# renegade-fi/renegade

Measured on AMD Instinct MI355X. Metric: VALID MATCH MPC proofs/sec (Intent And Balance Private Settlement), higher is better.
Workload: dtype u256; 1 GPU; intent_and_balance_private_settlement_proof; domain_n=4096, num_public=17, srs_power=13, prover_mode=cohort (lockstep rounds, fused per-round MSMs), total_proofs=4752, parallelism=x1 gpus, cohort=48, 4 in flight

## Files before the change

### renegade_amd/csrc/lagrange_kernels.hip

```cpp
#include <hip/hip_runtime.h>
#include "gpu_curve.hpp"
#include "msm_digits.hpp"

namespace rng {

struct Canon4 {
    uint64_t l[4];
};

__device__ inline G1Jac g1_mul_canon(const G1Jac& p, const uint64_t s[4]) {
    int top = -1;
    for (int i = 3; i >= 0 && top < 0; --i)
        if (s[i]) top = 64 * i + 63 - __clzll((long long)s[i]);
    G1Jac acc = G1Jac::identity();
    for (int bit = top; bit >= 0; --bit) {
        acc = acc.dbl();
        if ((s[bit >> 6] >> (bit & 63)) & 1) acc = acc.add(p);
    }
    return acc;
}

__global__ __launch_bounds__(256) void k_g1_ntt_load(const G1Aff* srs, uint32_t n,
                                                     G1Jac* pts) {
    uint32_t i = blockIdx.x * blockDim.x + threadIdx.x;
    if (i >= n) return;
    pts[i] = G1Jac::from_affine(srs[i]);
}

__global__ __launch_bounds__(64) void k_g1_ntt_pass(G1Jac* pts, uint32_t n, uint32_t h,
                                                    const Fr* tw) {
    uint32_t t = blockIdx.x * blockDim.x + threadIdx.x;
    if (t >= n / 2) return;
    uint32_t blk = t / h, j = t - blk * h;
    uint32_t i0 = blk * 2 * h + j, i1 = i0 + h;
    G1Jac a = pts[i0], b = pts[i1];
    pts[i0] = a.add(b);
    b.Y = b.Y.neg();
    G1Jac d = a.add(b);
    if (j != 0) {
        uint64_t s[4];
        tw[j * (n / (2 * h))].to_canonical(s);
        d = g1_mul_canon(d, s);
    }
    pts[i1] = d;
}

__global__ __launch_bounds__(64) void k_g1_ntt_finish(const G1Jac* in, const G1Aff* srs,
                                                      uint32_t n, uint32_t logn,
                                                      Canon4 ninv, G1Jac* out) {
    uint32_t i = blockIdx.x * blockDim.x + threadIdx.x;
    if (i >= n + 2) return;
    if (i >= n) {
        out[i] = G1Jac::from_affine(srs[i]).madd(srs[i - n], true);
        return;
    }
    uint32_t r = __brev(i) >> (32 - logn);
    out[i] = g1_mul_canon(in[r], ninv.l);
}

constexpr uint32_t LAG_NORM = 8;

__global__ __launch_bounds__(64) void k_g1_normalize(const G1Jac* pts, uint32_t N,
                                                     G1Aff* out, uint32_t* bad) {
    uint32_t t = blockIdx.x * blockDim.x + threadIdx.x;
    uint32_t lo = t * LAG_NORM;
    if (lo >= N) return;
    uint32_t cnt = N - lo < LAG_NORM ? N - lo : LAG_NORM;
    Fq pref[LAG_NORM];
    Fq run = Fq::one();
    for (uint32_t j = 0; j < cnt; ++j) {
        Fq z = pts[lo + j].Z;
        if (z.is_zero()) {
            atomicOr(bad, 1u);
            return;
        }
        run = run.mul(z);
        pref[j] = run;
    }
    Fq inv = run.inverse();
    for (int j = (int)cnt - 1; j >= 0; --j) {
        G1Jac p = pts[lo + j];
        Fq zinv = j ? inv.mul(pref[j - 1]) : inv;
        inv = inv.mul(p.Z);
        Fq zinv2 = zinv.sqr();
        G1Aff a;
        a.x = p.X.mul(zinv2);
        a.y = p.Y.mul(zinv2.mul(zinv));
        out[lo + j] = a;
    }
}


template <typename F>
__device__ inline void msm_signed_digits(const uint64_t s[4], uint32_t c, uint32_t W, F f) {
    uint32_t carry = 0;
    for (uint32_t w = 0; w < W; ++w) {
        MsmDigit d = msm_recode_digit(s, c, w, carry);
        if (d.mag) f(w, d.mag, d.sign);
    }
}

__global__ __launch_bounds__(256) void k_msm_digit_count(const uint64_t* scalars,
                                                         uint32_t total_scalars, uint32_t c,
                                                         uint32_t W, uint32_t* counts) {
    uint32_t idx = blockIdx.x * blockDim.x + threadIdx.x;
    if (idx >= total_scalars) return;
    uint64_t s[4] = {scalars[4 * idx], scalars[4 * idx + 1], scalars[4 * idx + 2],
                     scalars[4 * idx + 3]};
    uint32_t cnt = 0;
    if (s[0] | s[1] | s[2] | s[3])
        msm_signed_digits(s, c, W, [&](uint32_t, uint32_t, uint32_t) { ++cnt; });
    counts[idx] = cnt;
}

__global__ __launch_bounds__(256) void k_msm_digits_compact(
    const uint64_t* scalars, uint32_t n, uint32_t c, uint32_t W, uint32_t B, uint32_t N,
    const uint32_t* offs, uint32_t* keys, uint32_t* vals) {
    uint32_t idx = blockIdx.x * blockDim.x + threadIdx.x;
    if (idx >= n * B) return;
    uint64_t s[4] = {scalars[4 * idx], scalars[4 * idx + 1], scalars[4 * idx + 2],
                     scalars[4 * idx + 3]};
    if (!(s[0] | s[1] | s[2] | s[3])) return;
    uint32_t b = idx / n, i = idx % n;
    uint32_t o = offs[idx];
    msm_signed_digits(s, c, W, [&](uint32_t w, uint32_t mag, uint32_t sign) {
        keys[o] = (b << c) | mag;
        vals[o] = (sign << 31) | (w * N + i);
        ++o;
    });
}

__global__ __launch_bounds__(256) void k_count_nonzero_scalars(const uint64_t* scalars,
                                                               uint32_t total,
                                                               uint32_t* out) {
    uint32_t idx = blockIdx.x * blockDim.x + threadIdx.x;
    bool nz = false;
    if (idx < total)
        nz = (scalars[4 * idx] | scalars[4 * idx + 1] | scalars[4 * idx + 2] |
              scalars[4 * idx + 3]) != 0;
    uint32_t cnt = (uint32_t)__popcll(__ballot(nz));
    if ((threadIdx.x & 63) == 0 && cnt) atomicAdd(out, cnt);
}

__global__ __launch_bounds__(256) void k_lagrange_scalars(const Fr* evals,
                                                          const Fr* blinders, uint32_t n,
                                                          uint64_t total ,
                                                          uint64_t* out) {
    uint64_t i = (uint64_t)blockIdx.x * blockDim.x + threadIdx.x;
    if (i >= total) return;
    uint64_t g = i / (n + 2);
    uint32_t j = (uint32_t)(i - g * (n + 2));
    Fr v = j < n ? evals[g * n + j] : (blinders ? blinders[2 * g + (j - n)] : Fr::zero());
    v.to_canonical(out + 4 * i);
}

}
```

### renegade_amd/csrc/msm_digits.hpp

```cpp
#pragma once
#include <cstdint>

#if defined(__HIPCC__)
#define MSM_DIGIT_HD __host__ __device__
#else
#define MSM_DIGIT_HD
#endif

namespace rng {

struct MsmDigit {
    uint32_t mag;
    uint32_t sign;
};

MSM_DIGIT_HD inline MsmDigit msm_recode_digit(const uint64_t s[4], uint32_t c, uint32_t w,
                                              uint32_t& carry) {
    const uint32_t half = 1u << (c - 1);
    const uint64_t cmask = (1ull << c) - 1;
    const uint32_t bit0 = w * c;
    const uint32_t limb = bit0 >> 6, off = bit0 & 63;
    uint64_t raw = limb < 4 ? s[limb] >> off : 0;
    if (off + c > 64 && limb + 1 < 4) raw |= s[limb + 1] << (64 - off);
    raw = (raw & cmask) + carry;
    MsmDigit d;
    if (raw > half) {
        d.mag = (uint32_t)((1ull << c) - raw);
        d.sign = 1;
        carry = 1;
    } else {
        d.mag = (uint32_t)raw;
        d.sign = 0;
        carry = 0;
    }
    return d;
}

}
```

### renegade_amd/csrc/prover_api.hip

```cpp
#include <array>
#include <atomic>
#include <chrono>
#include <condition_variable>
#include <cstdio>
#include <functional>
#include <cstdlib>
#include <cstring>
#include <map>
#include <memory>
#include <mutex>
#include <stdexcept>
#include <thread>
#include <vector>

#include "../../include/rng_prover.h"
#include "ntt_kernels.hip"
#include "msm_kernels.hip"
#include "lagrange_kernels.hip"
#include "plonk_kernels.hip"
#include "perm_kernels.hip"
#include "open_kernels.hip"
#include "plonk_circuit.hpp"
#include "plonk_host.hpp"
#include "plonk_rounds.hpp"
// ... 39 lines not shown
    struct Job {
        std::function<void(uint32_t)> fn;
        uint32_t count;
        std::atomic<uint32_t> next{0}, done{0};
    };

  public:
    static HostPool& inst() {
        static HostPool* p = new HostPool();
        return *p;
    }

    void parallel_for(uint32_t count, const std::function<void(uint32_t)>& fn) {
        if (count == 0) return;
        if (count == 1 || workers_.empty()) {
            for (uint32_t i = 0; i < count; ++i) fn(i);
            return;
        }
        std::unique_lock<std::mutex> job_lk(job_mu_);
        auto job = std::make_shared<Job>();
        job->fn = fn;
        job->count = count;
        {
            std::lock_guard<std::mutex> lk(mu_);
            job_ = job;
            ++generation_;
        }
        cv_.notify_all();
        run_job(*job);
        {
            std::unique_lock<std::mutex> lk(mu_);
            done_cv_.wait(lk, [&] {
                return job->done.load(std::memory_order_acquire) >= count;
            });
            job_.reset();
        }
    }

  private:
    HostPool() {
        unsigned n = std::thread::hardware_concurrency();
        if (n == 0) n = 4;
        if (n > 32) n = 32;
        for (unsigned t = 0; t + 1 < n; ++t)
            workers_.emplace_back([this] { worker_loop(); });
    }
    void run_job(Job& job) {
        for (;;) {
            uint32_t i = job.next.fetch_add(1, std::memory_order_relaxed);
            if (i >= job.count) break;
            job.fn(i);
            if (job.done.fetch_add(1, std::memory_order_acq_rel) + 1 >= job.count) {
                std::lock_guard<std::mutex> lk(mu_);
                done_cv_.notify_all();
            }
        }
    }
    void worker_loop() {
        uint64_t seen = 0;
        for (;;) {
            std::shared_ptr<Job> job;
            {
                std::unique_lock<std::mutex> lk(mu_);
                cv_.wait(lk, [&] { return generation_ != seen || stopping_; });
                if (stopping_) return;
                seen = generation_;
                job = job_;
            }
            if (job) run_job(*job);
        }
    }
    std::mutex job_mu_;
    std::mutex mu_;
    std::condition_variable cv_, done_cv_;
    std::vector<std::thread> workers_;
    std::shared_ptr<Job> job_;
    uint64_t generation_ = 0;
    bool stopping_ = false;

  public:
    void stop() {
        std::unique_lock<std::mutex> job_lk(job_mu_);
        {
            std::lock_guard<std::mutex> lk(mu_);
            if (stopping_) return;
            stopping_ = true;
        }
        cv_.notify_all();
        for (auto& t : workers_) t.join();
        workers_.clear();
    }
};

struct EvtTimer {
    hipEvent_t ev[8];
    int used = 0;
    EvtTimer() {
        for (auto& e : ev) hipEventCreate(&e);
    }
    ~EvtTimer() {
        for (auto& e : ev) hipEventDestroy(e);
    }
    void mark(hipStream_t s) {
        if (used < 8) hipEventRecord(ev[used++], s);
    }
    void collect(double* out, int n) {
        hipEventSynchronize(ev[used - 1]);
        for (int i = 0; i < n && i + 1 < used; ++i) {
            float ms = 0;
            hipEventElapsedTime(&ms, ev[i], ev[i + 1]);
            out[i] = ms;
        }
    }
};


struct NttPlan {
    uint32_t n, logn, N1, N2, logN1, logN2, split_log;
    Fr *wst1_f = nullptr, *wst2_f = nullptr, *ta_f = nullptr, *tb_f = nullptr;
    Fr *wst1_i = nullptr, *wst2_i = nullptr, *ta_i = nullptr, *tb_i = nullptr;
    Fr ninv;
    Fr* scratch = nullptr;
    uint64_t scratch_elems = 0;
    Fr *gpow = nullptr, *gpow_inv = nullptr, *xpow = nullptr;
};

static Fr h_fr_root_of_unity(uint32_t n) {
    static const u64 root_c[4] = FR_TWO_ADIC_ROOT;
    Fr root = Fr::from_canonical(root_c);
    uint32_t logn = 0;
    while ((1u << logn) < n) logn++;
    for (uint32_t i = logn; i < FR_TWO_ADICITY; ++i) root = root.sqr();
    return root;
}

struct RngCtxImpl {
    std::vector<uint64_t> srs_g1_host;
    uint64_t srs_count = 0;
    void* srs_dev = nullptr;
    struct FixedTable {
        uint32_t c = 0;
        void* dev = nullptr;
    };
    FixedTable fixed_tables[3];
    struct LookupTable {
        void* dev = nullptr;
        bool tried = false;
    };
    LookupTable lookup_tables[3];
    struct LagrangeDomain {
        bool usable = false;
        void* bases = nullptr;
        FixedTable tables[2];
    };
    std::map<uint64_t, LagrangeDomain> lagrange;
    uint64_t h_g2[16];
    uint64_t beta_h_g2[16];
    std::map<uint32_t, std::unique_ptr<NttPlan>> plans;
    std::mutex mu;

    ~RngCtxImpl() {
        for (auto& kv : plans) {
            NttPlan* p = kv.second.get();
            for (Fr* b : {p->wst1_f, p->wst2_f, p->ta_f, p->tb_f, p->wst1_i,
                          p->wst2_i, p->ta_i, p->tb_i, p->scratch, p->gpow,
                          p->gpow_inv, p->xpow})
                hip_free_guarded(b);
        }
        hip_free_guarded(srs_dev);
        for (auto& t : fixed_tables) hip_free_guarded(t.dev);
        for (auto& t : lookup_tables) hip_free_guarded(t.dev);
        for (auto& kv : lagrange) {
            hip_free_guarded(kv.second.bases);
            for (auto& t : kv.second.tables) hip_free_guarded(t.dev);
        }
    }
};

static int build_pow_table(Fr** out, const Fr& base, uint64_t step, uint64_t count) {
    HIP_CHECK(hipMalloc(out, count * sizeof(Fr)));
    uint32_t blocks = (uint32_t)((count + 255) / 256);
    hipLaunchKernelGGL(k_pow_table, dim3(blocks), dim3(256), 0, 0, *out, base, step, count);
    HIP_CHECK(hipGetLastError());
    return RNG_OK;
}

static constexpr uint32_t NTT_SMALL_MAX = 1024;
static constexpr uint64_t NTT_MAX_N = 1ull << 24;
static constexpr bool NTT_FILL_DEFAULT = true;

static bool ntt_args_ok(uint64_t n, uint64_t batch) {
    return n >= 2 && !(n & (n - 1)) && n <= NTT_MAX_N && batch >= 1;
}

static NttPlan* get_plan(RngCtxImpl* ctx, uint32_t n, uint64_t batch) {
    std::lock_guard<std::mutex> lk(ctx->mu);
    auto it = ctx->plans.find(n);
    NttPlan* p;
    if (it != ctx->plans.end()) {
        p = it->second.get();
    } else {
        auto np = std::make_unique<NttPlan>();
        p = np.get();
        p->n = n;
        p->logn = 0;
        while ((1u << p->logn) < n) p->logn++;
        p->logN2 = p->logn / 2;
        p->logN1 = p->logn - p->logN2;
        p->N1 = 1u << p->logN1;
        p->N2 = 1u << p->logN2;
        p->split_log = p->logN2 < 6 ? p->logN2 : 6;
        Fr w = h_fr_root_of_unity(n);
        Fr wi = w.inverse();
        Fr wN1_f = w.pow_u64(p->N2), wN2_f = w.pow_u64(p->N1);
        Fr wN1_i = wi.pow_u64(p->N2), wN2_i = wi.pow_u64(p->N1);
        uint64_t split = 1ull << p->split_log;
        if (n <= NTT_SMALL_MAX) {
            if (build_pow_table(&p->wst1_f, w, 1, n / 2) != RNG_OK) return nullptr;
            if (build_pow_table(&p->wst1_i, wi, 1, n / 2) != RNG_OK) return nullptr;
        } else {
            if (build_pow_table(&p->wst1_f, wN1_f, 1, p->N1 / 2) != RNG_OK) return nullptr;
            if (build_pow_table(&p->wst2_f, wN2_f, 1, p->N2 / 2) != RNG_OK) return nullptr;
            if (build_pow_table(&p->ta_f, w, split, (uint64_t)p->N1 * (p->N2 >> p->split_log)) != RNG_OK) return nullptr;
            if (build_pow_table(&p->tb_f, w, 1, (uint64_t)p->N1 * split) != RNG_OK) return nullptr;
            if (build_pow_table(&p->wst1_i, wN1_i, 1, p->N1 / 2) != RNG_OK) return nullptr;
            if (build_pow_table(&p->wst2_i, wN2_i, 1, p->N2 / 2) != RNG_OK) return nullptr;
            if (build_pow_table(&p->ta_i, wi, split, (uint64_t)p->N1 * (p->N2 >> p->split_log)) != RNG_OK) return nullptr;
            if (build_pow_table(&p->tb_i, wi, 1, (uint64_t)p->N1 * split) != RNG_OK) return nullptr;
        }
        u64 nc[4] = {n, 0, 0, 0};
        p->ninv = Fr::from_canonical(nc).inverse();
        if (hipDeviceSynchronize() != hipSuccess) return nullptr;
        ctx->plans.emplace(n, std::move(np));
    }
    if (n > NTT_SMALL_MAX && p->scratch_elems < (uint64_t)n * batch) {
        if (p->scratch) hipFree(p->scratch);
        if (hipMalloc(&p->scratch, (uint64_t)n * batch * sizeof(Fr)) != hipSuccess) {
            p->scratch = nullptr;
            p->scratch_elems = 0;
            return nullptr;
        }
        p->scratch_elems = (uint64_t)n * batch;
    }
    return p;
}

static int ntt_dev_run(RngCtxImpl* ctx, Fr* data, Fr* out, uint32_t n, uint64_t batch,
                       bool inverse, hipStream_t stream = 0) {
    NttPlan* p = get_plan(ctx, n, 0);
    if (!p) return RNG_ERR_HIP;
    if (n <= NTT_SMALL_MAX) {
        Fr* wst = inverse ? p->wst1_i : p->wst1_f;
        hipLaunchKernelGGL(k_ntt_small, dim3((uint32_t)batch), dim3(512), n * sizeof(Fr),
                           stream, data, wst, n, p->logn, p->ninv, inverse ? 1 : 0);
        HIP_CHECK(hipGetLastError());
        if (out != data)
            HIP_CHECK(hipMemcpyAsync(out, data, (uint64_t)n * batch * sizeof(Fr),
                                     hipMemcpyDeviceToDevice, stream));
        return RNG_OK;
    }
    Fr* wst1 = inverse ? p->wst1_i : p->wst1_f;
    Fr* wst2 = inverse ? p->wst2_i : p->wst2_f;
    Fr* ta = inverse ? p->ta_i : p->ta_f;
    Fr* tb = inverse ? p->tb_i : p->tb_f;
    static uint32_t pw_lds_cap = [] {
        const char* e = getenv("RNG_NTT_PAIR_LDS");
        return e ? (uint32_t)atoi(e) : 65536u;
    }();
    static const bool fill = [] {
        const char* e = getenv("RNG_NTT_FILL");
        return e ? atoi(e) != 0 : NTT_FILL_DEFAULT;
    }();
    const uint32_t fpw1 = NTT_FILL_ELEMS / p->N2, fpw2 = NTT_FILL_ELEMS / p->N1;
    const bool fill1 = fill && fpw1 >= 2 && fpw1 <= p->N1;
    const bool fill2 = fill && fpw2 >= 2 && fpw2 <= p->N2;
    const uint32_t pw1 = (2u * p->N2 * sizeof(Fr) <= pw_lds_cap) ? 2 : 1;
    const uint32_t pw2 = (2u * p->N1 * sizeof(Fr) <= pw_lds_cap) ? 2 : 1;
    uint32_t lds1 = pw1 * p->N2 * sizeof(Fr);
    uint32_t lds2 = pw2 * p->N1 * sizeof(Fr);
    EvtTimer et;
    et.mark(stream);
    if (fill1)
        hipLaunchKernelGGL(k_ntt_col_fill, dim3((uint32_t)(p->N1 / fpw1 * batch)),
                           dim3(NTT_FILL_THREADS), NTT_FILL_ELEMS * sizeof(Fr), stream, data,
                           wst2, ta, tb, p->N1, p->N2, p->logN2, p->split_log,
                           (uint32_t)__builtin_ctz(fpw1));
    else if (pw1 == 2)
        hipLaunchKernelGGL(k_ntt_col<2>, dim3((uint32_t)(p->N1 / 2 * batch)), dim3(512),
                           lds1, stream, data, wst2, ta, tb, p->N1, p->N2, p->logN2,
                           p->split_log);
    else
        hipLaunchKernelGGL(k_ntt_col<1>, dim3((uint32_t)(p->N1 * batch)), dim3(512),
                           lds1, stream, data, wst2, ta, tb, p->N1, p->N2, p->logN2,
                           p->split_log);
    HIP_CHECK(hipGetLastError());
    et.mark(stream);
    if (fill2)
        hipLaunchKernelGGL(k_ntt_row_fill, dim3((uint32_t)(p->N2 / fpw2 * batch)),
                           dim3(NTT_FILL_THREADS), NTT_FILL_ELEMS * sizeof(Fr), stream, data,
                           out, wst1, p->N1, p->N2, p->logN1, (uint32_t)__builtin_ctz(fpw2),
                           p->ninv, inverse ? 1 : 0);
    else if (pw2 == 2)
        hipLaunchKernelGGL(k_ntt_row<2>, dim3((uint32_t)(p->N2 / 2 * batch)), dim3(512),
                           lds2, stream, data, out, wst1, p->N1, p->N2, p->logN1,
                           p->ninv, inverse ? 1 : 0);
    else
        hipLaunchKernelGGL(k_ntt_row<1>, dim3((uint32_t)(p->N2 * batch)), dim3(512),
                           lds2, stream, data, out, wst1, p->N1, p->N2, p->logN1,
                           p->ninv, inverse ? 1 : 0);
    HIP_CHECK(hipGetLastError());
    et.mark(stream);
    et.collect(tls_ntt_times, 2);
    return RNG_OK;
}


struct MsmEnv {
    int fixed;
    int c;
    int chunk;
    int subb;
    int seg_cap;
    int debug;
    int lookup;
    int lookup_max_mb;
    int lookup_c;
    int lookup_l;
};

static const MsmEnv& msm_env() {
    static const MsmEnv env = [] {
        auto get = [](const char* name, int unset) {
            const char* e = getenv(name);
            return e ? atoi(e) : unset;
        };
        return MsmEnv{get("RNG_MSM_FIXED", 1),  get("RNG_MSM_C", 0),
                      get("RNG_MSM_CHUNK", 0),  get("RNG_MSM_SUBB", 0),
                      get("RNG_MSM_SEGCAP", 0), get("RNG_MSM_DEBUG", 0),
                      get("RNG_MSM_LOOKUP", -1), get("RNG_MSM_LOOKUP_MAX_MB", 10240),
                      get("RNG_MSM_LOOKUP_C", 0), get("RNG_MSM_LOOKUP_L", 0)};
    }();
    return env;
}

struct ProverEnv {
    int z_device;
    int r1_lagrange;
    int open_device;
    int cohort_trace;
    static bool on(int v, bool path_default) { return v < 0 ? path_default : v == 1; }
};

static const ProverEnv& prover_env() {
    static const ProverEnv env = [] {
        auto tri = [](const char* name) {
            const char* e = getenv(name);
            return e ? (atoi(e) != 0 ? 1 : 0) : -1;
        };
        const char* t = getenv("RNG_COHORT_TRACE");
        return ProverEnv{tri("RNG_Z_DEVICE"), tri("RNG_R1_LAGRANGE"), tri("RNG_OPEN_DEVICE"),
                         t ? atoi(t) : 0};
    }();
    return env;
}

struct MsmBases {
    const G1Aff* points;
    uint64_t table_stride;
    static MsmBases plain(const G1Aff* bases) { return {bases, 0}; }
    static MsmBases table(const G1Aff* t, uint64_t stride) { return {t, stride}; }
    bool fixed() const { return table_stride != 0; }
};

struct MsmShape {
    uint64_t n;
    uint32_t B, c;
    bool fixed;
    bool compact;
    uint32_t Wd;
    uint32_t W;
    uint32_t G;
    uint32_t key_shift;
    uint64_t total;
    uint64_t nb;
    uint32_t chunk_sz;
    uint64_t nchunks;
    uint32_t cw;
    uint32_t subb;
    uint32_t seg_cap;
    uint32_t sentinel;
    uint32_t sort_bits;
};

static MsmShape msm_shape(uint64_t n, uint32_t B, uint32_t c, bool fixed,
                          bool compact = false) {
    const MsmEnv& env = msm_env();
    MsmShape sh;
    sh.n = n;
    sh.B = B;
    sh.c = c;
    sh.fixed = fixed;
    sh.compact = compact;
    sh.Wd = (256 + c - 1) / c;
    sh.W = fixed ? 1 : sh.Wd;
    sh.G = B * sh.W;
    sh.key_shift = fixed ? c : 16;
    sh.total = n * B * sh.Wd;
    sh.nb = (1ull << (c - 1)) * sh.G;
    sh.chunk_sz = MSM_CHUNK;
    while (sh.chunk_sz > 2 && sh.nb / sh.chunk_sz < 131072) sh.chunk_sz >>= 1;
    if (env.chunk >= 2 && env.chunk <= 16) sh.chunk_sz = (uint32_t)env.chunk;
    if ((1u << (c - 1)) < sh.chunk_sz) sh.chunk_sz = 1u << (c - 1);
    sh.nchunks = ((1ull << (c - 1)) / sh.chunk_sz) * sh.G;
    sh.cw = (1u << (c - 1)) / sh.chunk_sz;
    sh.subb = MSM_SUBB;
    while (sh.subb > 1 && sh.cw / sh.subb < 64) sh.subb >>= 1;
    while (sh.subb < 256 && sh.G * sh.subb < 4096 && sh.cw / (2 * sh.subb) >= 64 &&
           (uint64_t)sh.G * sh.subb * 2 <= 8192)
        sh.subb <<= 1;
    if (env.subb >= 1 && env.subb <= 256) sh.subb = (uint32_t)env.subb;
    sh.seg_cap = msm_seg_cap(sh.total);
    if (fixed && env.seg_cap >= 8 && env.seg_cap <= (int)MSM_MAX_SEG)
        sh.seg_cap = (uint32_t)env.seg_cap;
    uint32_t gb = 1;
    while ((1u << gb) <= sh.G) ++gb;
    sh.sentinel = sh.G << sh.key_shift;
    sh.sort_bits = sh.key_shift + gb;
    return sh;
}

struct MsmScratch {
    uint32_t *keys_in = nullptr, *keys_out = nullptr, *vals_in = nullptr, *vals_out = nullptr;
    void* sort_temp = nullptr;
    size_t sort_temp_bytes = 0;
    uint8_t* head_flags = nullptr;
    uint32_t* heads = nullptr;
    uint32_t* lens = nullptr;
    uint32_t* nsub = nullptr;
    uint32_t* sub_off = nullptr;
    uint32_t* sub_start = nullptr;
    uint32_t* sub_len = nullptr;
    uint32_t* sub_len_sorted = nullptr;
    uint32_t* sub_order = nullptr;
    uint32_t* nsub_sorted = nullptr;
    uint32_t* head_order = nullptr;
    G1Jac* partials2 = nullptr;
    uint32_t* head_count = nullptr;
    void* select_temp = nullptr;
    size_t select_temp_bytes = 0;
    void* scan_temp = nullptr;
    size_t scan_temp_bytes = 0;
    G1Jac* buckets = nullptr;
    G1Jac* partials = nullptr;
    G1Jac* window_sums = nullptr;
    uint64_t window_sums_cap = 0;
    G1Jac* result = nullptr;
    uint64_t cap_entries = 0;
    uint64_t cap_nb = 0;
    uint64_t cap_nchunks = 0;
    uint64_t last_entries = 0;

    ~MsmScratch() {
        for (void* b : {(void*)keys_in, (void*)keys_out, (void*)vals_in, (void*)vals_out,
                        sort_temp, (void*)head_flags, (void*)heads, (void*)lens,
                        (void*)nsub, (void*)sub_off, (void*)sub_start, (void*)sub_len,
                        (void*)sub_len_sorted, (void*)sub_order,
                        (void*)nsub_sorted, (void*)head_order,
                        (void*)partials2, (void*)head_count, select_temp, scan_temp,
                        (void*)buckets, (void*)partials, (void*)window_sums,
                        (void*)result})
            hip_free_guarded(b);
    }
};

static thread_local std::unique_ptr<MsmScratch> tls_msm_scratch;

static int msm_scratch_ensure(const MsmShape& sh, hipStream_t stream, MsmScratch** out) {
    if (!tls_msm_scratch) tls_msm_scratch = std::make_unique<MsmScratch>();
    MsmScratch* s = tls_msm_scratch.get();
    if (s->cap_entries < sh.total || s->cap_nb < sh.nb || s->cap_nchunks < sh.nchunks) {
        uint64_t cap_total = sh.total + sh.total / 2 + 64;
        uint64_t cap_nb2 = sh.nb + sh.nb / 2 + 64;
        uint64_t cap_nch = sh.nchunks + sh.nchunks / 2 + 64;
        if (cap_total < s->cap_entries) cap_total = s->cap_entries;
        if (cap_nb2 < s->cap_nb) cap_nb2 = s->cap_nb;
        if (cap_nch < s->cap_nchunks) cap_nch = s->cap_nchunks;
        tls_msm_scratch = std::make_unique<MsmScratch>();
        s = tls_msm_scratch.get();
        HIP_CHECK(hipMalloc(&s->keys_in, cap_total * 4));
        HIP_CHECK(hipMalloc(&s->keys_out, cap_total * 4));
        HIP_CHECK(hipMalloc(&s->vals_in, cap_total * 4));
        HIP_CHECK(hipMalloc(&s->vals_out, cap_total * 4));
        rocprim::radix_sort_pairs(nullptr, s->sort_temp_bytes, s->keys_in, s->keys_out,
// ... 376 lines not shown
    tls_msm_times[2] = ms;
    MsmShape sh{};
    sh.B = sh.G = B;
    sh.W = 1;
    sh.subb = bpp;
    sh.c = c;
    msm_host_fold(sh, wsums, h_result);
    return RNG_OK;
}

static int msm_srs_run(RngCtxImpl* ctx, const uint64_t* d_canon, uint64_t m, uint32_t B,
                       G1Jac* res, int window_c = 0, int mode = 0) {
    if (m == 0 || m > ctx->srs_count || B == 0) return RNG_ERR_BAD_ARG;
    const int c_env = msm_env().c;
    if (window_c == 0 && c_env >= 8 && c_env <= 16) window_c = c_env;
    if (window_c != 0 && (window_c < 8 || window_c > 16)) return RNG_ERR_BAD_ARG;
    if (mode == 3 || (mode == 0 && msm_fixed_enabled() && msm_lookup_wanted(B))) {
        uint32_t c = (uint32_t)window_c;
        const G1Aff* table = nullptr;
        if (B <= 65535)
            table = window_c ? msm_lookup_table(ctx, c) : msm_lookup_select(ctx, &c);
        if (table) return msm_lookup_run(table, ctx->srs_count, d_canon, m, c, res, B);
        if (mode == 3) return RNG_ERR_BAD_ARG;
    }
    if (mode == 1 || (mode == 0 && msm_fixed_enabled())) {
        uint32_t c = window_c ? (uint32_t)window_c : msm_fixed_c(m, B);
        uint32_t gb = 1;
        while ((1u << gb) <= B) ++gb;
        const G1Aff* table = (c + gb <= 32) ? msm_fixed_table(ctx, c) : nullptr;
        if (table)
            return msm_dev_run(MsmBases::table(table, ctx->srs_count), d_canon, m, c, res,
                               B);
        if (mode == 1) return RNG_ERR_BAD_ARG;
    }
    uint32_t c = window_c ? (uint32_t)window_c : msm_auto_c(m);
    if ((uint64_t)B * ((256 + c - 1) / c) > 60000) return RNG_ERR_BAD_ARG;
    return msm_dev_run(MsmBases::plain((const G1Aff*)ctx->srs_dev), d_canon, m, c, res, B);
}


constexpr int MSM_LAGRANGE_UNUSABLE = -100;

static int lagrange_build_bases(RngCtxImpl* ctx, uint64_t n, void** out_bases) {
    const uint32_t N = (uint32_t)n + 2;
    uint32_t logn = 0;
    while ((1ull << logn) < n) ++logn;
    const hipStream_t st = RNG_STREAM;
    G1Jac *pts = nullptr, *fin = nullptr;
    Fr* tw = nullptr;
    uint32_t* bad = nullptr;
    void* bases = nullptr;
    auto cleanup = [&] {
        hipFree(pts);
        hipFree(fin);
        hipFree(tw);
        hipFree(bad);
    };
    if (hipMalloc(&pts, n * sizeof(G1Jac)) != hipSuccess ||
        hipMalloc(&fin, (uint64_t)N * sizeof(G1Jac)) != hipSuccess ||
        hipMalloc(&tw, (n / 2) * sizeof(Fr)) != hipSuccess ||
        hipMalloc(&bad, 4) != hipSuccess ||
        hipMalloc(&bases, (uint64_t)N * sizeof(G1Aff)) != hipSuccess) {
        cleanup();
        hipFree(bases);
        return RNG_ERR_HIP;
    }
    const Fr winv = h_fr_root_of_unity((uint32_t)n).inverse();
    Fr nfr = Fr::one();
    for (uint32_t i = 0; i < logn; ++i) nfr = nfr.add(nfr);
    Canon4 ninv;
    nfr.inverse().to_canonical(ninv.l);
    const G1Aff* srs = (const G1Aff*)ctx->srs_dev;
    hipMemsetAsync(bad, 0, 4, st);
    hipLaunchKernelGGL(k_pow_table, dim3((uint32_t)((n / 2 + 255) / 256)), dim3(256), 0, st,
                       tw, winv, (uint64_t)1, n / 2);
    hipLaunchKernelGGL(k_g1_ntt_load, dim3((uint32_t)((n + 255) / 256)), dim3(256), 0, st,
                       srs, (uint32_t)n, pts);
    for (uint32_t h = (uint32_t)n / 2; h >= 1; h >>= 1)
        hipLaunchKernelGGL(k_g1_ntt_pass, dim3((uint32_t)((n / 2 + 63) / 64)), dim3(64), 0,
                           st, pts, (uint32_t)n, h, (const Fr*)tw);
    hipLaunchKernelGGL(k_g1_ntt_finish, dim3((N + 63) / 64), dim3(64), 0, st,
                       (const G1Jac*)pts, srs, (uint32_t)n, logn, ninv, fin);
    const uint32_t norm_threads = (N + LAG_NORM - 1) / LAG_NORM;
    hipLaunchKernelGGL(k_g1_normalize, dim3((norm_threads + 63) / 64), dim3(64), 0, st,
                       (const G1Jac*)fin, N, (G1Aff*)bases, bad);
    uint32_t h_bad = 1;
    bool ok = hipGetLastError() == hipSuccess &&
              hipMemcpyAsync(&h_bad, bad, 4, hipMemcpyDeviceToHost, st) == hipSuccess &&
              hipStreamSynchronize(st) == hipSuccess;
    cleanup();
    if (!ok || h_bad) {
        hipFree(bases);
        return ok ? MSM_LAGRANGE_UNUSABLE : RNG_ERR_HIP;
    }
    *out_bases = bases;
    return RNG_OK;
}

static const G1Aff* msm_lagrange_table(RngCtxImpl* ctx, uint64_t n, uint32_t c) {
    if (!ctx->srs_dev || n < 2 || (n & (n - 1)) || n > (1ull << 28) ||
        n + 2 > ctx->srs_count || c < 8 || c > 16)
        return nullptr;
    const uint64_t N = n + 2;
    const uint32_t W = (256 + c - 1) / c;
    if ((uint64_t)W * N * sizeof(G1Aff) > (1ull << 30)) return nullptr;
    static const int trace = msm_env().debug;
    std::lock_guard<std::mutex> lk(ctx->mu);
    auto it = ctx->lagrange.find(n);
    if (it == ctx->lagrange.end()) {
        auto t0 = std::chrono::steady_clock::now();
        RngCtxImpl::LagrangeDomain dom;
        dom.usable = lagrange_build_bases(ctx, n, &dom.bases) == RNG_OK;
        it = ctx->lagrange.emplace(n, dom).first;
        if (trace)
            fprintf(stderr, "[lagrange] n=%lu bases %s in %.2f ms\n", (unsigned long)n,
                    dom.usable ? "built" : "UNUSABLE",
                    std::chrono::duration<double, std::milli>(
                        std::chrono::steady_clock::now() - t0).count());
    }
    RngCtxImpl::LagrangeDomain& dom = it->second;
    if (!dom.usable) return nullptr;
    for (auto& t : dom.tables)
        if (t.dev && t.c == c) return (const G1Aff*)t.dev;
    for (auto& t : dom.tables) {
        if (t.dev) continue;
        auto t0 = std::chrono::steady_clock::now();
        void* dev = nullptr;
        if (hipMalloc(&dev, (uint64_t)W * N * sizeof(G1Aff)) != hipSuccess) return nullptr;
        hipLaunchKernelGGL(k_msm_fixed_table, dim3((uint32_t)((N + 255) / 256)), dim3(256),
                           0, RNG_STREAM, (const G1Aff*)dom.bases, (uint32_t)N, c, W,
                           (G1Aff*)dev);
        if (hipGetLastError() != hipSuccess ||
            hipStreamSynchronize(RNG_STREAM) != hipSuccess) {
            hipFree(dev);
            return nullptr;
        }
        t.c = c;
        t.dev = dev;
        if (trace)
            fprintf(stderr, "[lagrange] n=%lu c=%u table (%.1f MB) in %.2f ms\n",
                    (unsigned long)n, c, (double)W * N * sizeof(G1Aff) / 1e6,
                    std::chrono::duration<double, std::milli>(
                        std::chrono::steady_clock::now() - t0).count());
        return (const G1Aff*)dev;
    }
    return nullptr;
}

constexpr uint32_t MSM_LAGRANGE_SPARSE_C = 8, MSM_LAGRANGE_DENSE_C = 13;
static uint32_t msm_lagrange_c(uint64_t n, uint32_t B, uint64_t nonzero) {
    return nonzero * 2 <= (uint64_t)B * n ? MSM_LAGRANGE_SPARSE_C : 0;
}

static int msm_lagrange_run(RngCtxImpl* ctx, uint64_t n, const uint64_t* d_canon, uint32_t B,
                            G1Jac* res, int window_c = 0, bool dense_too = false) {
    if (n < 2 || (n & (n - 1)) || B == 0 || !d_canon) return RNG_ERR_BAD_ARG;
    if (n + 2 > ctx->srs_count) return MSM_LAGRANGE_UNUSABLE;
    const int c_env = msm_env().c;
    if (window_c == 0 && c_env >= 8 && c_env <= 16) window_c = c_env;
    if (window_c != 0 && (window_c < 8 || window_c > 16)) return RNG_ERR_BAD_ARG;
    uint32_t c = (uint32_t)window_c;
    if (c == 0) {
        MsmScratch* s = nullptr;
        int rc = msm_scratch_ensure(msm_shape(n + 2, B, 8, true, true), RNG_STREAM, &s);
        if (rc != RNG_OK) return rc;
        const uint32_t ns = (uint32_t)(B * (n + 2));
        uint32_t nz = 0;
        HIP_CHECK(hipMemsetAsync(s->head_count, 0, 4, RNG_STREAM));
        hipLaunchKernelGGL(k_count_nonzero_scalars, dim3((ns + 255) / 256), dim3(256), 0,
                           RNG_STREAM, d_canon, ns, s->head_count);
        HIP_CHECK(hipGetLastError());
        HIP_CHECK(hipMemcpyAsync(&nz, s->head_count, 4, hipMemcpyDeviceToHost, RNG_STREAM));
        HIP_CHECK(hipStreamSynchronize(RNG_STREAM));
        c = msm_lagrange_c(n, B, nz);
        if (c == 0) {
            if (!dense_too) return MSM_LAGRANGE_UNUSABLE;
            c = MSM_LAGRANGE_DENSE_C;
        }
    }
    uint32_t gb = 1;
    while ((1u << gb) <= B) ++gb;
    if (c + gb > 32) return MSM_LAGRANGE_UNUSABLE;
    const G1Aff* table = msm_lagrange_table(ctx, n, c);
    if (!table) return MSM_LAGRANGE_UNUSABLE;
    return msm_dev_run(MsmBases::table(table, n + 2), d_canon, n + 2, c, res, B, RNG_STREAM,
                       true);
}

constexpr uint32_t R1_LAGRANGE_MIN_K = 2;


static int ensure_coset_tables(RngCtxImpl* ctx, NttPlan* p) {
    std::lock_guard<std::mutex> lk(ctx->mu);
    if (p->gpow) return RNG_OK;
    uint32_t m = p->n;
    Fr g = Fr::from_u64(FR_GENERATOR);
    Fr gi = g.inverse();
    if (build_pow_table(&p->gpow, g, 1, m) != RNG_OK) return RNG_ERR_HIP;
    if (build_pow_table(&p->gpow_inv, gi, 1, m) != RNG_OK) return RNG_ERR_HIP;
    Fr wm = h_fr_root_of_unity(m);
    if (build_pow_table(&p->xpow, wm, 1, m) != RNG_OK) return RNG_ERR_HIP;
    uint32_t blocks = (m + 255) / 256;
    hipLaunchKernelGGL(k_scale_const, dim3(blocks), dim3(256), 0, 0, p->xpow, g, m);
    HIP_CHECK(hipGetLastError());
    HIP_CHECK(hipDeviceSynchronize());
    return RNG_OK;
}

static int coset_fwd_dev(RngCtxImpl* ctx, Fr* in, Fr* out, uint32_t m) {
    NttPlan* p = get_plan(ctx, m, 1);
    if (!p) return RNG_ERR_HIP;
    if (ensure_coset_tables(ctx, p) != RNG_OK) return RNG_ERR_HIP;
    uint32_t blocks = (m + 255) / 256;
    hipLaunchKernelGGL(k_mul_pointwise, dim3(blocks), dim3(256), 0, RNG_STREAM, in,
                       p->gpow, m);
    HIP_CHECK(hipGetLastError());
    return ntt_dev_run(ctx, in, out, m, 1, false, RNG_STREAM);
}

struct ProveScratch {
    static constexpr uint32_t SLOTS = 13;
    uint64_t n = 0;
    Fr* tmp = nullptr;
    Fr* stage = nullptr;
    uint64_t* canon = nullptr;
    ~ProveScratch() {
        for (void* b : {(void*)tmp, (void*)stage, (void*)canon}) hip_free_guarded(b);
    }
};

struct PlonkPkImpl : PlonkPkHost {
    Fr* sel_coset = nullptr;
    Fr* sig_coset = nullptr;
    Fr* l1_coset = nullptr;
    Fr* sig_evals_dev = nullptr;
    Fr* wpow_dev = nullptr;
    Fr* coef_dev = nullptr;
    RngCtxImpl* ctx = nullptr;
    ~PlonkPkImpl() {
        for (void* b : {(void*)sel_coset, (void*)sig_coset, (void*)l1_coset,
                        (void*)sig_evals_dev, (void*)wpow_dev, (void*)coef_dev})
            hip_free_guarded(b);
    }
};

static thread_local std::unique_ptr<ProveScratch> tls_prove_scratch;

static int prove_scratch_ensure(uint64_t n) {
    if (tls_prove_scratch && tls_prove_scratch->n >= n) return RNG_OK;
    tls_prove_scratch = std::make_unique<ProveScratch>();
    ProveScratch* s = tls_prove_scratch.get();
    HIP_CHECK(hipMalloc(&s->tmp, 8 * n * sizeof(Fr)));
    HIP_CHECK(hipMalloc(&s->stage, ProveScratch::SLOTS * (n + 3) * sizeof(Fr)));
    HIP_CHECK(hipMalloc(&s->canon, ProveScratch::SLOTS * 4 * (n + 3) * 8));
    s->n = n;
    return RNG_OK;
}


constexpr bool Z_DEVICE_DEFAULT = true;

static void perm_product_host(const PlonkPkImpl& pk, const Fr& w, const Fr* wires,
                              const Fr& beta, const Fr& gamma, Fr* ze) {
    const uint64_t n = pk.n;
    std::vector<Fr> znum(n), zden(n);
    Fr wi = Fr::one();
    for (uint64_t i = 0; i < n; ++i) {
        Fr num = Fr::one(), den = Fr::one();
        for (int j = 0; j < 5; ++j) {
            Fr wv = wires[(size_t)j * n + i];
            num = num.mul(wv.add(beta.mul(pk.k[j]).mul(wi)).add(gamma));
            den = den.mul(wv.add(beta.mul(pk.sig_evals[j][i])).add(gamma));
        }
        znum[i] = num;
        zden[i] = den;
        wi = wi.mul(w);
    }
    std::vector<Fr> zden_inv = hbatch_inverse(zden);
    ze[0] = Fr::one();
    for (uint64_t i = 1; i < n; ++i) ze[i] = ze[i - 1].mul(znum[i - 1]).mul(zden_inv[i - 1]);
}

struct PermScratch {
    Fr* dev = nullptr;
    Fr* tile_tot = nullptr;
    Fr* tile_pre = nullptr;
    Fr* totals = nullptr;
    Fr* qinv = nullptr;
    Fr* bg = nullptr;
    std::vector<Fr> h_bg, h_q;
    ~PermScratch() { hip_free_guarded(dev); }
};

static thread_local std::unique_ptr<PermScratch> tls_perm_scratch;

static PermScratch* perm_scratch_get() {
    if (tls_perm_scratch) return tls_perm_scratch.get();
    auto s = std::make_unique<PermScratch>();
    const size_t tiles = (size_t)2 * PERM_MAX_BATCH * PERM_MAX_TILES;
    const size_t elems = 2 * tiles + 5 * (size_t)PERM_MAX_BATCH;
    if (hipMalloc(&s->dev, elems * sizeof(Fr)) != hipSuccess) return nullptr;
    s->tile_tot = s->dev;
    s->tile_pre = s->tile_tot + tiles;
    s->totals = s->tile_pre + tiles;
    s->qinv = s->totals + 2 * PERM_MAX_BATCH;
    s->bg = s->qinv + PERM_MAX_BATCH;
    s->h_bg.resize(2 * PERM_MAX_BATCH);
    s->h_q.resize(PERM_MAX_BATCH);
    tls_perm_scratch = std::move(s);
    return tls_perm_scratch.get();
}

static int perm_product_dev(const Fr* wires, const Fr* sigma, const Fr* wpow,
                            const Fr k5[5], const Fr* bg, uint64_t n64, uint64_t batch64,
// ... 1669 lines not shown
```

Before: 3507 proofs/s.

## Add entry-lookup MSM path for sparse round-one Lagrange commitments

Adds a new MSM path for sparse Lagrange-basis commitments. Each nonzero signed digit is looked up in a precomputed multiples table indexed by (window row, magnitude) and mixed-added directly, which removes bucket sorting and bucket reduction. The digit count and the nonzero-density check are fused into one kernel with block-level atomics, so a separate count pass is no longer needed. The cost is a large cached lookup table in device memory, an extra host sync, and a host-side fold of per-block partial sums.

New measurement: 3800 proofs/s (median of 6 runs). 1.08x the previous value.

```diff
diff --git a/renegade_amd/csrc/lagrange_kernels.hip b/renegade_amd/csrc/lagrange_kernels.hip
--- a/renegade_amd/csrc/lagrange_kernels.hip
+++ b/renegade_amd/csrc/lagrange_kernels.hip
@@ -100,6 +100,17 @@
     }
 }
 
+__device__ inline void block_count_add(bool flag, uint32_t* out) {
+    __shared__ uint32_t wave_cnt[4];
+    const uint32_t cnt = (uint32_t)__popcll(__ballot(flag));
+    if ((threadIdx.x & 63) == 0) wave_cnt[threadIdx.x >> 6] = cnt;
+    __syncthreads();
+    if (threadIdx.x == 0) {
+        const uint32_t sum = wave_cnt[0] + wave_cnt[1] + wave_cnt[2] + wave_cnt[3];
+        if (sum) atomicAdd(out, sum);
+    }
+}
+
 __global__ __launch_bounds__(256) void k_msm_digit_count(const uint64_t* scalars,
                                                          uint32_t total_scalars, uint32_t c,
                                                          uint32_t W, uint32_t* counts) {
@@ -113,6 +124,21 @@
     counts[idx] = cnt;
 }
 
+__global__ __launch_bounds__(256) void k_msm_digit_count_density(
+    const uint64_t* scalars, uint32_t total_scalars, uint32_t c, uint32_t W, uint32_t* counts,
+    uint32_t* nonzero) {
+    uint32_t idx = blockIdx.x * blockDim.x + threadIdx.x;
+    uint32_t cnt = 0;
+    if (idx < total_scalars) {
+        uint64_t s[4] = {scalars[4 * idx], scalars[4 * idx + 1], scalars[4 * idx + 2],
+                         scalars[4 * idx + 3]};
+        if (s[0] | s[1] | s[2] | s[3])
+            msm_signed_digits(s, c, W, [&](uint32_t, uint32_t, uint32_t) { ++cnt; });
+    }
+    if (idx <= total_scalars) counts[idx] = cnt;
+    block_count_add(cnt != 0, nonzero);
+}
+
 __global__ __launch_bounds__(256) void k_msm_digits_compact(
     const uint64_t* scalars, uint32_t n, uint32_t c, uint32_t W, uint32_t B, uint32_t N,
     const uint32_t* offs, uint32_t* keys, uint32_t* vals) {
@@ -124,8 +150,8 @@
     uint32_t b = idx / n, i = idx % n;
     uint32_t o = offs[idx];
     msm_signed_digits(s, c, W, [&](uint32_t w, uint32_t mag, uint32_t sign) {
-        keys[o] = (b << c) | mag;
-        vals[o] = (sign << 31) | (w * N + i);
+        keys[o] = msm_entry_key(b, mag, c);
+        vals[o] = msm_entry_val(w, N, i, sign);
         ++o;
     });
 }
@@ -138,8 +164,37 @@
     if (idx < total)
         nz = (scalars[4 * idx] | scalars[4 * idx + 1] | scalars[4 * idx + 2] |
               scalars[4 * idx + 3]) != 0;
-    uint32_t cnt = (uint32_t)__popcll(__ballot(nz));
-    if ((threadIdx.x & 63) == 0 && cnt) atomicAdd(out, cnt);
+    block_count_add(nz, out);
+}
+
+__global__ __launch_bounds__(256) void k_msm_entry_lookup_sum(
+    const uint32_t* keys, const uint32_t* vals, const uint32_t* offs, uint32_t N, uint32_t c,
+    const G1Aff* table, G1Jac* partials) {
+    __shared__ G1Jac red[256];
+    const uint32_t b = blockIdx.y;
+    const uint32_t lo = offs[(uint64_t)b * N], hi = offs[(uint64_t)(b + 1) * N];
+    const uint32_t first = blockIdx.x * 256;
+    G1Jac* out = partials + (uint64_t)b * gridDim.x + blockIdx.x;
+    if (first >= hi - lo) {
+        if (threadIdx.x == 0) *out = G1Jac::identity();
+        return;
+    }
+    const uint32_t active = hi - lo - first < 256 ? hi - lo - first : 256;
+    const uint64_t step = (uint64_t)gridDim.x * 256;
+    G1Jac acc = G1Jac::identity();
+    for (uint64_t e = (uint64_t)lo + first + threadIdx.x; e < hi; e += step) {
+        const uint32_t key = keys[e], val = vals[e];
+        const G1Aff p = table[msm_lookup_index(key, val, c)];
+        acc = acc.madd(p, msm_entry_sign(val) != 0);
+    }
+    red[threadIdx.x] = acc;
+    __syncthreads();
+    for (uint32_t stride = 128; stride > 0; stride >>= 1) {
+        if (threadIdx.x < stride && threadIdx.x + stride < active)
+            red[threadIdx.x] = red[threadIdx.x].add(red[threadIdx.x + stride]);
+        __syncthreads();
+    }
+    if (threadIdx.x == 0) *out = red[0];
 }
 
 __global__ __launch_bounds__(256) void k_lagrange_scalars(const Fr* evals,
diff --git a/renegade_amd/csrc/msm_digits.hpp b/renegade_amd/csrc/msm_digits.hpp
--- a/renegade_amd/csrc/msm_digits.hpp
+++ b/renegade_amd/csrc/msm_digits.hpp
@@ -36,4 +36,28 @@
     return d;
 }
 
+
+MSM_DIGIT_HD inline uint32_t msm_entry_key(uint32_t poly, uint32_t mag, uint32_t c) {
+    return (poly << c) | mag;
 }
+MSM_DIGIT_HD inline uint32_t msm_entry_val(uint32_t w, uint32_t N, uint32_t i, uint32_t sign) {
+    return (sign << 31) | (w * N + i);
+}
+MSM_DIGIT_HD inline uint32_t msm_entry_mag(uint32_t key, uint32_t c) {
+    return key & ((1u << c) - 1);
+}
+MSM_DIGIT_HD inline uint32_t msm_entry_row(uint32_t val) { return val & 0x7fffffffu; }
+MSM_DIGIT_HD inline uint32_t msm_entry_sign(uint32_t val) { return val >> 31; }
+
+MSM_DIGIT_HD inline uint64_t msm_table_rows(uint64_t N, uint32_t c) {
+    return (uint64_t)((256 + c - 1) / c) * N;
+}
+MSM_DIGIT_HD inline bool msm_entry_rows_fit(uint64_t N, uint32_t c) {
+    return msm_table_rows(N, c) < (1ull << 31);
+}
+
+MSM_DIGIT_HD inline uint64_t msm_lookup_index(uint32_t key, uint32_t val, uint32_t c) {
+    return ((uint64_t)msm_entry_row(val) << (c - 1)) + (msm_entry_mag(key, c) - 1);
+}
+
+}
diff --git a/renegade_amd/csrc/prover_api.hip b/renegade_amd/csrc/prover_api.hip
--- a/renegade_amd/csrc/prover_api.hip
+++ b/renegade_amd/csrc/prover_api.hip
@@ -215,6 +215,7 @@
         bool usable = false;
         void* bases = nullptr;
         FixedTable tables[2];
+        LookupTable lookup[3];
     };
     std::map<uint64_t, LagrangeDomain> lagrange;
     uint64_t h_g2[16];
@@ -236,6 +237,7 @@
         for (auto& kv : lagrange) {
             hip_free_guarded(kv.second.bases);
             for (auto& t : kv.second.tables) hip_free_guarded(t.dev);
+            for (auto& t : kv.second.lookup) hip_free_guarded(t.dev);
         }
     }
 };
@@ -389,6 +391,8 @@
     int lookup_max_mb;
     int lookup_c;
     int lookup_l;
+    int r1_lookup;
+    int r1_lookup_s;
 };
 
 static const MsmEnv& msm_env() {
@@ -401,7 +405,8 @@
                       get("RNG_MSM_CHUNK", 0),  get("RNG_MSM_SUBB", 0),
                       get("RNG_MSM_SEGCAP", 0), get("RNG_MSM_DEBUG", 0),
                       get("RNG_MSM_LOOKUP", -1), get("RNG_MSM_LOOKUP_MAX_MB", 10240),
-                      get("RNG_MSM_LOOKUP_C", 0), get("RNG_MSM_LOOKUP_L", 0)};
+                      get("RNG_MSM_LOOKUP_C", 0), get("RNG_MSM_LOOKUP_L", 0),
+                      get("RNG_R1_LOOKUP", -1), get("RNG_R1_LOOKUP_S", 0)};
     }();
     return env;
 }
@@ -1084,6 +1089,188 @@
     return nonzero * 2 <= (uint64_t)B * n ? MSM_LAGRANGE_SPARSE_C : 0;
 }
 
+
+constexpr bool R1_LOOKUP_DEFAULT = true;
+
+static bool r1_lookup_wanted(uint32_t B) {
+    const int sw = msm_env().r1_lookup;
+    return msm_lookup_wanted(B) && (sw < 0 ? R1_LOOKUP_DEFAULT : sw == 1);
+}
+
+static const G1Aff* msm_lagrange_lookup_table(RngCtxImpl* ctx, uint64_t n, uint32_t c) {
+    if (c < MSM_LOOKUP_MIN_C || c > MSM_LOOKUP_MAX_C) return nullptr;
+    const uint64_t N = n + 2;
+    const uint64_t bytes = msm_lookup_bytes(N, c);
+    const int max_mb = msm_env().lookup_max_mb;
+    if (max_mb <= 0 || bytes > ((uint64_t)max_mb << 20) || !msm_entry_rows_fit(N, c))
+        return nullptr;
+    {
+        std::lock_guard<std::mutex> lk(ctx->mu);
+        auto it = ctx->lagrange.find(n);
+        if (it != ctx->lagrange.end()) {
+            RngCtxImpl::LookupTable& t = it->second.lookup[c - MSM_LOOKUP_MIN_C];
+            if (t.dev || t.tried || !it->second.usable) return (const G1Aff*)t.dev;
+        }
+    }
+    const G1Aff* fixed = msm_lagrange_table(ctx, n, c);
+    if (!fixed) return nullptr;
+    std::lock_guard<std::mutex> lk(ctx->mu);
+    RngCtxImpl::LookupTable& t = ctx->lagrange.find(n)->second.lookup[c - MSM_LOOKUP_MIN_C];
+    if (t.dev || t.tried) return (const G1Aff*)t.dev;
+    t.tried = true;
+    size_t free_b = 0, total_b = 0;
+    if (hipMemGetInfo(&free_b, &total_b) != hipSuccess || bytes > free_b / 2) return nullptr;
+    const auto t0 = std::chrono::steady_clock::now();
+    void* dev = nullptr;
+    if (hipMalloc(&dev, bytes) != hipSuccess) {
+        (void)hipGetLastError();
+        return nullptr;
+    }
+    const uint64_t rows = msm_table_rows(N, c);
+    hipLaunchKernelGGL(k_msm_lookup_table, dim3((uint32_t)((rows + 255) / 256)), dim3(256), 0,
+                       RNG_STREAM, fixed, rows, c, (G1Aff*)dev);
+    if (hipGetLastError() != hipSuccess || hipStreamSynchronize(RNG_STREAM) != hipSuccess) {
+        hipFree(dev);
+        return nullptr;
+    }
+    if (msm_env().debug)
+        fprintf(stderr,
+                "[msm] lagrange lookup table n=%lu c=%u rows=%lu bytes=%lu build_ms=%.1f\n",
+                (unsigned long)n, c, (unsigned long)rows, (unsigned long)bytes,
+                std::chrono::duration<double, std::milli>(std::chrono::steady_clock::now() - t0)
+                    .count());
+    t.dev = dev;
+    return (const G1Aff*)dev;
+}
+
+struct R1LookupScratch {
+    uint32_t *counts = nullptr, *offs = nullptr;
+    uint64_t cap_scalars = 0;
+    void* scan_temp = nullptr;
+    size_t scan_temp_bytes = 0;
+    uint32_t *keys = nullptr, *vals = nullptr;
+    uint64_t cap_entries = 0;
+    G1Jac* partials = nullptr;
+    uint64_t cap_partials = 0;
+    ~R1LookupScratch() {
+        for (void* b : {(void*)counts, (void*)offs, scan_temp, (void*)keys, (void*)vals,
+                        (void*)partials})
+            hip_free_guarded(b);
+    }
+};
+static thread_local R1LookupScratch tls_r1_lookup;
+
+static int r1_scratch_grow(void** buf, uint64_t* cap, uint64_t want, size_t elem) {
+    if (*cap >= want) return RNG_OK;
+    hipFree(*buf);
+    *buf = nullptr;
+    *cap = 0;
+    const uint64_t ncap = want + want / 2 + 64;
+    HIP_CHECK(hipMalloc(buf, ncap * elem));
+    *cap = ncap;
+    return RNG_OK;
+}
+
+constexpr uint32_t R1_LOOKUP_PER_LANE = 4, R1_LOOKUP_MAX_S = 64;
+static uint32_t r1_lookup_blocks(uint64_t entries, uint32_t B) {
+    const int s_env = msm_env().r1_lookup_s;
+    if (s_env >= 1 && s_env <= (int)R1_LOOKUP_MAX_S) return (uint32_t)s_env;
+    const uint64_t per_block = 256ull * R1_LOOKUP_PER_LANE;
+    uint64_t S = (entries / B + per_block - 1) / per_block;
+    return (uint32_t)(S < 1 ? 1 : S > R1_LOOKUP_MAX_S ? R1_LOOKUP_MAX_S : S);
+}
+
+constexpr int R1_LOOKUP_DENSE = -101, R1_LOOKUP_NO_TABLE = -102;
+
+static int r1_lookup_run(RngCtxImpl* ctx, uint64_t n, const uint64_t* d_canon, uint32_t B,
+                         uint32_t c, bool gate, G1Jac* h_result) {
+    const hipStream_t stream = RNG_STREAM;
+    const uint32_t N = (uint32_t)n + 2, W = (256 + c - 1) / c;
+    const uint32_t ns = B * N;
+    {
+        std::lock_guard<std::mutex> lk(ctx->mu);
+        auto it = ctx->lagrange.find(n);
+        if (it != ctx->lagrange.end()) {
+            const RngCtxImpl::LookupTable& t = it->second.lookup[c - MSM_LOOKUP_MIN_C];
+            if (!it->second.usable || (t.tried && !t.dev)) return R1_LOOKUP_NO_TABLE;
+        }
+    }
+    R1LookupScratch& s = tls_r1_lookup;
+    if (s.cap_scalars < ns) {
+        uint64_t cap_c = s.cap_scalars, cap_o = s.cap_scalars;
+        int rc = r1_scratch_grow((void**)&s.counts, &cap_c, (uint64_t)ns + 2, 4);
+        if (rc == RNG_OK) rc = r1_scratch_grow((void**)&s.offs, &cap_o, (uint64_t)ns + 2, 4);
+        s.cap_scalars = 0;
+        if (rc != RNG_OK) return rc;
+        hipFree(s.scan_temp);
+        s.scan_temp = nullptr;
+        (void)rocprim::exclusive_scan(nullptr, s.scan_temp_bytes, s.counts, s.offs, 0u, cap_c,
+                                      rocprim::plus<uint32_t>(), stream);
+        HIP_CHECK(hipMalloc(&s.scan_temp, s.scan_temp_bytes));
+        s.cap_scalars = cap_c - 2;
+    }
+    EvtTimer et;
+    et.mark(stream);
+    HIP_CHECK(hipMemsetAsync(s.offs + ns + 1, 0, 4, stream));
+    hipLaunchKernelGGL(k_msm_digit_count_density, dim3(ns / 256 + 1), dim3(256), 0, stream,
+                       d_canon, ns, c, W, s.counts, s.offs + ns + 1);
+    HIP_CHECK(hipGetLastError());
+    (void)rocprim::exclusive_scan(s.scan_temp, s.scan_temp_bytes, s.counts, s.offs, 0u,
+                                  (size_t)ns + 1, rocprim::plus<uint32_t>(), stream);
+    et.mark(stream);
+    uint32_t back[2] = {0, 0};
+    HIP_CHECK(hipMemcpyAsync(back, s.offs + ns, 8, hipMemcpyDeviceToHost, stream));
+    HIP_CHECK(hipStreamSynchronize(stream));
+    const uint64_t entries = back[0];
+    if (gate && msm_lagrange_c(n, B, back[1]) == 0) return R1_LOOKUP_DENSE;
+    const G1Aff* table = msm_lagrange_lookup_table(ctx, n, c);
+    if (!table) return R1_LOOKUP_NO_TABLE;
+    const uint32_t S = r1_lookup_blocks(entries, B);
+    if (msm_env().debug)
+        fprintf(stderr, "[msm] n=%lu B=%u entry-lookup c=%u S=%u entries=%lu (compacted)\n",
+                (unsigned long)N, B, c, S, (unsigned long)entries);
+    for (double& t : tls_msm_times) t = 0;
+    if (entries == 0) {
+        for (uint32_t b = 0; b < B; ++b) h_result[b] = G1Jac::identity();
+        et.collect(tls_msm_times, 1);
+        return RNG_OK;
+    }
+    const uint64_t np = (uint64_t)B * S;
+    int rc = r1_scratch_grow((void**)&s.partials, &s.cap_partials, np, sizeof(G1Jac));
+    if (rc != RNG_OK) return rc;
+    if (s.cap_entries < entries) {
+        uint64_t cap_k = s.cap_entries, cap_v = s.cap_entries;
+        rc = r1_scratch_grow((void**)&s.keys, &cap_k, entries, 4);
+        if (rc == RNG_OK) rc = r1_scratch_grow((void**)&s.vals, &cap_v, entries, 4);
+        s.cap_entries = rc == RNG_OK ? cap_k : 0;
+        if (rc != RNG_OK) return rc;
+    }
+    et.mark(stream);
+    hipLaunchKernelGGL(k_msm_digits_compact, dim3((ns + 255) / 256), dim3(256), 0, stream,
+                       d_canon, N, c, W, B, N, s.offs, s.keys, s.vals);
+    HIP_CHECK(hipGetLastError());
+    et.mark(stream);
+    hipLaunchKernelGGL(k_msm_entry_lookup_sum, dim3(S, B), dim3(256), 0, stream, s.keys,
+                       s.vals, s.offs, N, c, table, s.partials);
+    HIP_CHECK(hipGetLastError());
+    et.mark(stream);
+    std::vector<G1Jac> wsums((size_t)np);
+    HIP_CHECK(hipMemcpyAsync(wsums.data(), s.partials, np * sizeof(G1Jac),
+                             hipMemcpyDeviceToHost, stream));
+    HIP_CHECK(hipStreamSynchronize(stream));
+    double ms[4] = {0, 0, 0, 0};
+    et.collect(ms, 4);
+    tls_msm_times[0] = ms[0] + ms[2];
+    tls_msm_times[2] = ms[3];
+    MsmShape sh{};
+    sh.B = sh.G = B;
+    sh.W = 1;
+    sh.subb = S;
+    sh.c = c;
+    msm_host_fold(sh, wsums, h_result);
+    return RNG_OK;
+}
+
 static int msm_lagrange_run(RngCtxImpl* ctx, uint64_t n, const uint64_t* d_canon, uint32_t B,
                             G1Jac* res, int window_c = 0, bool dense_too = false) {
     if (n < 2 || (n & (n - 1)) || B == 0 || !d_canon) return RNG_ERR_BAD_ARG;
@@ -1092,6 +1279,18 @@
     if (window_c == 0 && c_env >= 8 && c_env <= 16) window_c = c_env;
     if (window_c != 0 && (window_c < 8 || window_c > 16)) return RNG_ERR_BAD_ARG;
     uint32_t c = (uint32_t)window_c;
+    const uint32_t c_try = c ? c : MSM_LAGRANGE_SPARSE_C;
+    if (r1_lookup_wanted(B) && c_try >= MSM_LOOKUP_MIN_C && c_try <= MSM_LOOKUP_MAX_C &&
+        B <= 65535 && msm_table_rows(n + 2, c_try) * B < (1ull << 32)) {
+        int rc = r1_lookup_run(ctx, n, d_canon, B, c_try, c == 0, res);
+        if (rc != R1_LOOKUP_DENSE && rc != R1_LOOKUP_NO_TABLE) return rc;
+        if (rc == R1_LOOKUP_DENSE) {
+            if (!dense_too) return MSM_LAGRANGE_UNUSABLE;
+            c = MSM_LAGRANGE_DENSE_C;
+        } else {
+            c = c_try;
+        }
+    }
     if (c == 0) {
         MsmScratch* s = nullptr;
         int rc = msm_scratch_ensure(msm_shape(n + 2, B, 8, true, true), RNG_STREAM, &s);
```
